# Research-Implementation/AudioVidSum-A-Multi-Modal-Approach-to-Video-Summarization

Hardware: AMD Instinct MI355X
Metric: frames/sec end-to-end (extract+fuse+score), 224x224 + 16kHz (higher is better)
Workload: dtype f16x2; 1 GPU; configs[1]: SumMe-shape batch, 25 videos x ~1800 frames (45143 frames/GPU), visual-only resnet50 extractor (batch-stat BN, the reference's 4-frame BatchNorm micro-batches inside each video) + AVBiLSTM attention scorer + mean-threshold selection; frames_per_gpu=45143, videos_per_gpu=25, extractor=resnet50, frames_per_group=4, chunk_frames=16384, parallelism=videos sharded x1, no data-path collective, selected_frames_rank0=22823

## Files before the change

audiovidsum-a-multi-modal-approach-to-video-summarization_amd/csrc/local224.hip:

```cpp
#include "avs_internal.h"
#include "igemm_params.h"
#include <type_traits>
#include <utility>

namespace {
constexpr int L_ROWS = 224;
constexpr int L_MT = L_ROWS / 32;
constexpr int L_BN = 128;
constexpr int L_CPRR = 4;
constexpr int L_STEP = 16;
constexpr int L_BUF = (L_ROWS + L_BN) * L_CPRR;
constexpr int L_P = 32 + 8;
constexpr unsigned L_OOB = 0x80000000u;

template <int OFF>
__device__ __forceinline__ uint4 lds_read_b128_at(unsigned byte_addr) {
  uint4 v;
  asm volatile("ds_read_b128 %0, %1 offset:%2" : "=v"(v) : "v"(byte_addr), "n"(OFF));
  return v;
}
template <int... I>
__device__ __forceinline__ void read_blocks(uint4 (&f)[L_MT], unsigned addr, std::integer_sequence<int, I...>) {
  ((f[I] = lds_read_b128_at<I * 32 * 64>(addr)), ...);
}
}

template <bool SPATIAL>
__global__ __launch_bounds__(256, 2) void igemm_h2_local224_kernel(IgemmParams p) {
  __shared__ uint4 lds[3 * L_BUF];

  const unsigned nwg = gridDim.x, orig = blockIdx.x;
  const unsigned q = nwg >> 3, rr = nwg & 7, xcd = orig & 7;
  const unsigned wg = (xcd < rr ? xcd * (q + 1) : rr * (q + 1) + (xcd - rr) * q) + (orig >> 3);
  int tn = wg % p.tiles_n;
  int tm = wg / p.tiles_n;
  if (p.packed) {
    const unsigned u_t = (unsigned)p.packed, tnn = (unsigned)p.tiles_n;
    const unsigned tiles_m = nwg / tnn;
    const unsigned full = (56u % u_t == 0u) ? (tiles_m / 56u) * 56u : 0u;
    if (orig < full * tnn) {
      const unsigned su = orig / (56u * tnn), l = orig - su * (56u * tnn);
      tn = (int)(l / 56u);
      tm = (int)(su * 56u + l % 56u);
    } else {
      const unsigned o2 = orig - full * tnn, unit = u_t * tnn;
      const unsigned u = o2 / unit, l = o2 - u * unit;
      const unsigned left = tiles_m - full - u * u_t, ul = left < u_t ? left : u_t;
      tn = (int)(l / ul);
      tm = (int)(full + u * u_t + l % ul);
    }
  } else if (p.cluster > 1) {
    const unsigned c = (unsigned)p.cluster, tnn = (unsigned)p.tiles_n;
    const unsigned tiles_m = nwg / tnn;
    const unsigned full = (8u % c == 0u) ? (tiles_m / 8u) * 8u : 0u;
    if (orig < full * tnn) {
      const unsigned su = orig / (8u * tnn), l = orig - su * (8u * tnn);
      tn = (int)(l >> 3);
      tm = (int)(su * 8u + (l & 7u));
    } else {
      const unsigned o2 = orig - full * tnn, unit = c * tnn;
      const unsigned u = o2 / unit, l = o2 - u * unit;
      tn = (int)(l / c);
      tm = (int)(full + u * c + l % c);
    }
  }
  const int m0 = tm * p.tile_rows;
  const int n0 = tn * L_BN;
  const int used = m0 + p.tile_rows <= p.M ? p.tile_rows : p.M - m0;

  const char* __restrict__ x = p.x;
  const char* __restrict__ w = p.w;
  char* __restrict__ y = p.y;

  const int t = threadIdx.x;
  const int wave = __builtin_amdgcn_readfirstlane(t >> 6), lane = t & 63;
  const bool extra = wave < 2;
  const int c = t & (L_CPRR - 1);
  const int rb = t >> 2;
  const int cq = c ^ ((rb >> 2) & (L_CPRR - 1));

  unsigned amask[4], aoff[4], boff[2];
  int f_tap = 0, f_ci0 = 0, f_kw = 0;
  int f_koff = 0;
  int f_kb = 0;
  __amdgpu_buffer_rsrc_t a_rsrc, b_rsrc;
  {
    const int taps = p.K / p.cin;
    long long a_origin;
    int n_first = 0;
    if (p.lin_stride >= 0) {
      a_origin = (long long)m0 * p.lin_stride;
    } else {
      n_first = m0 / p.HoWo;
      a_origin = (long long)n_first * p.x_img_stride - (long long)p.ph * p.x_row_stride - (long long)p.pw * p.x_px_stride;
    }
    a_rsrc = __builtin_amdgcn_make_buffer_rsrc(const_cast<char*>(x) + a_origin * 4, 0, (int)L_OOB, 0x00020000);
    b_rsrc = __builtin_amdgcn_make_buffer_rsrc(
        const_cast<char*>(w) + (p.w_kstep ? (long long)n0 * 64 : (long long)n0 * p.ldb * 4), 0, (int)L_OOB, 0x00020000);
#pragma unroll
    for (int i = 0; i < 4; ++i) {
      unsigned mk = 0, off = L_OOB;
      const int r = rb + 64 * i;
      if (r < used) {
        const int m = m0 + r;
        if (p.lin_stride >= 0) {
          mk = ~0u;
          off = (unsigned)((long long)r * p.lin_stride * 4) + cq * 16;
        } else {
          const int n = m / p.HoWo;
          const int rem = m - n * p.HoWo;
          const int ho = rem / p.Wo;
          const int wo = rem - ho * p.Wo;
          const int hi0 = ho * p.sh - p.ph, wi0 = wo * p.sw - p.pw;
          if constexpr (SPATIAL) {
            for (int tp = 0; tp < taps; ++tp) {
              const int th = tp / p.KW, tw = tp - th * p.KW;
              if ((unsigned)(hi0 + th) < (unsigned)p.H && (unsigned)(wi0 + tw) < (unsigned)p.W) mk |= 1u << tp;
            }
          } else {
            mk = ~0u;
          }
          off = (unsigned)(((long long)(n - n_first) * p.x_img_stride + (long long)(hi0 + p.ph) * p.x_row_stride +
                            (long long)(wi0 + p.pw) * p.x_px_stride) * 4) + cq * 16;
        }
      }
      amask[i] = mk;
      aoff[i] = off;
    }
#pragma unroll
    for (int i = 0; i < 2; ++i)
      boff[i] = p.w_kstep ? (unsigned)((rb + 64 * i) * 64) + (unsigned)(cq >> 2) * (unsigned)p.N * 64u + (cq & 3) * 16
                          : (unsigned)((long long)(rb + 64 * i) * p.ldb * 4) + cq * 16;
  }

  auto stage = [&](int buf) {
    uint4* abuf = lds + buf * L_BUF + wave * 64;
    uint4* bbuf = abuf + L_ROWS * L_CPRR;
#pragma unroll
    for (int i = 0; i < 3; ++i) {
      unsigned off = aoff[i];
      if constexpr (SPATIAL) off = ((amask[i] >> f_tap) & 1u) ? off : L_OOB;
      __builtin_amdgcn_raw_ptr_buffer_load_lds(a_rsrc, (__attribute__((address_space(3))) void*)(abuf + 256 * i), 16,
                                               (int)off, f_koff, 0, 0);
    }
    if (extra) {
      unsigned off = aoff[3];
      if constexpr (SPATIAL) off = ((amask[3] >> f_tap) & 1u) ? off : L_OOB;
      __builtin_amdgcn_raw_ptr_buffer_load_lds(a_rsrc, (__attribute__((address_space(3))) void*)(abuf + 256 * 3), 16,
                                               (int)off, f_koff, 0, 0);
    }
#pragma unroll
    for (int i = 0; i < 2; ++i)
      __builtin_amdgcn_raw_ptr_buffer_load_lds(b_rsrc, (__attribute__((address_space(3))) void*)(bbuf + 256 * i), 16,
                                               (int)boff[i], f_kb, 0, 0);
    f_kb += p.w_kstep ? p.N * 64 : L_STEP * 4;
    f_ci0 += L_STEP;
    f_koff += L_STEP * 4;
    if (f_ci0 == p.cin) {
      f_ci0 = 0;
      ++f_tap;
      f_koff += (int)((p.x_px_stride - p.cin) * 4);
      if (++f_kw == p.KW) {
        f_kw = 0;
        f_koff += (int)((p.x_row_stride - (long long)p.KW * p.x_px_stride) * 4);
      }
    }
  };

  const int lr = lane & 31, lh = lane >> 5;

  f32x16 acc[L_MT];
#pragma unroll
  for (int i = 0; i < L_MT; ++i)
#pragma unroll
    for (int e = 0; e < 16; ++e) acc[i][e] = 0.f;

  const unsigned lds_base = (unsigned)(unsigned long long)((__attribute__((address_space(3))) char*)lds);
  unsigned fa_off[2], fb_off[2];
#pragma unroll
  for (int hl = 0; hl < 2; ++hl) {
    const int chunk = 2 * lh + hl;
    fa_off[hl] = (unsigned)(lr * L_CPRR + (chunk ^ ((lr >> 2) & (L_CPRR - 1)))) * 16u;
    const int brow = wave * 32 + lr;
    fb_off[hl] = (unsigned)((L_ROWS + brow) * L_CPRR + (chunk ^ ((brow >> 2) & (L_CPRR - 1)))) * 16u;
  }

  const int col = n0 + wave * 32 + lr;
  const float inv_n = 1.f / (float)p.tile_rows;
  const int lim = used - 4 * lh;
  const int rl0 = lane >> 2, grp = lane & 3;
  const int col8 = n0 + wave * 32 + grp * 8;
  constexpr int DEPTH = 6;
  uint4 rhi[DEPTH][2], rlo[DEPTH][2];
  auto res_fetch = [&](auto blk) {
    constexpr int mt = decltype(blk)::value;
    const long long row0 = (long long)m0 + mt * 32 + rl0;
    const char* base = p.residual + (row0 * p.ldr + col8) * 4;
#pragma unroll
    for (int it = 0; it < 2; ++it) {
      const bool ok = mt * 32 + rl0 + 16 * it < used;
      const uint4* rp = reinterpret_cast<const uint4*>(ok ? base + (long long)it * 16 * p.ldr * 4 : p.residual);
      rhi[mt % DEPTH][it] = rp[0];
      rlo[mt % DEPTH][it] = rp[1];
    }
  };
  if (p.residual) {
    res_fetch(std::integral_constant<int, 0>{});
    res_fetch(std::integral_constant<int, 1>{});
    res_fetch(std::integral_constant<int, 2>{});
  }

  const int steps = p.K / L_STEP;
  stage(0);
  if (steps > 1) stage(1);
  int cur = 0;
  for (int s = 0; s < steps; ++s) {
    if (s + 1 < steps) {
      if (extra)
        asm volatile("s_waitcnt vmcnt(6)" ::: "memory");
      else
        asm volatile("s_waitcnt vmcnt(5)" ::: "memory");
    } else {
      asm volatile("s_waitcnt vmcnt(0)" ::: "memory");
    }
    __builtin_amdgcn_s_barrier();
    const unsigned bbase = lds_base + (unsigned)cur * (L_BUF * 16u);
    uint4 fah[L_MT], fal[L_MT], fbh, fbl;
    fbh = avs_lds_read_b128(bbase + fb_off[0]);
    read_blocks(fah, bbase + fa_off[0], std::make_integer_sequence<int, L_MT>{});
    fbl = avs_lds_read_b128(bbase + fb_off[1]);
    read_blocks(fal, bbase + fa_off[1], std::make_integer_sequence<int, L_MT>{});
    if (s + 2 < steps) stage(cur == 0 ? 2 : cur - 1);
    asm volatile("s_waitcnt lgkmcnt(%0)" ::"n"(1 + L_MT) : "memory");
    avs_pin(fbh);
#pragma unroll
    for (int mt = 0; mt < L_MT; ++mt) avs_pin(fah[mt]);
    __builtin_amdgcn_sched_barrier(0);
#pragma unroll
    for (int mt = 0; mt < L_MT; ++mt)
      acc[mt] = __builtin_amdgcn_mfma_f32_32x32x16_f16(__builtin_bit_cast(avs_f16x8, fah[mt]),
                                                       __builtin_bit_cast(avs_f16x8, fbh), acc[mt], 0, 0, 0);
    asm volatile("s_waitcnt lgkmcnt(0)" ::: "memory");
    avs_pin(fbl);
#pragma unroll
    for (int mt = 0; mt < L_MT; ++mt) avs_pin(fal[mt]);
    __builtin_amdgcn_sched_barrier(0);
#pragma unroll
    for (int mt = 0; mt < L_MT; ++mt) {
      acc[mt] = __builtin_amdgcn_mfma_f32_32x32x16_f16(__builtin_bit_cast(avs_f16x8, fal[mt]),
                                                       __builtin_bit_cast(avs_f16x8, fbh), acc[mt], 0, 0, 0);
      acc[mt] = __builtin_amdgcn_mfma_f32_32x32x16_f16(__builtin_bit_cast(avs_f16x8, fah[mt]),
                                                       __builtin_bit_cast(avs_f16x8, fbl), acc[mt], 0, 0, 0);
    }
    __builtin_amdgcn_sched_barrier(0);
    cur = cur == 2 ? 0 : cur + 1;
  }

  if (p.residual) {
    res_fetch(std::integral_constant<int, 3>{});
    res_fetch(std::integral_constant<int, 4>{});
    res_fetch(std::integral_constant<int, 5>{});
  }
  const int seg0 = p.packed ? (int)min((long long)used, (m0 / p.rows_per_group + 1ll) * p.rows_per_group - m0) : used;
  const bool shared = seg0 < used;
  float mean, mean_b, s2, s2b = 0.f;
  if (p.packed) {
    float s1 = 0.f, s1b = 0.f;
#pragma unroll
    for (int mt = 0; mt < L_MT; ++mt)
#pragma unroll
      for (int e = 0; e < 16; ++e) {
        if (mt < 3 || (mt == 3 && e < 8))
          s1 += acc[mt][e];
        else
          s1b += acc[mt][e];
      }
    s1 += __shfl_xor(s1, 32, 64);
    s1b += __shfl_xor(s1b, 32, 64);
    const float inv0 = 1.f / (float)seg0, inv1 = 1.f / (float)(shared ? used - seg0 : seg0);
    mean = (shared ? s1 : s1 + s1b) * inv0;
    mean_b = shared ? s1b * inv1 : mean;
    s2 = 0.f;
#pragma unroll
    for (int mt = 0; mt < L_MT; ++mt)
#pragma unroll
      for (int e = 0; e < 16; ++e) {
        const int roff = mt * 32 + (e & 3) + 8 * (e >> 2);
        if (mt < 3 || (mt == 3 && e < 8)) {
          const float d = acc[mt][e] - mean;
          s2 = roff < lim ? fmaf(d, d, s2) : s2;
        } else {
          const float d = acc[mt][e] - mean_b;
          s2b = roff < lim ? fmaf(d, d, s2b) : s2b;
        }
      }
    s2 += __shfl_xor(s2, 32, 64);
    s2b += __shfl_xor(s2b, 32, 64);
    if (!shared) s2 += s2b;
  } else {
    float s1 = 0.f;
#pragma unroll
    for (int mt = 0; mt < L_MT; ++mt)
#pragma unroll
      for (int e = 0; e < 16; ++e) s1 += acc[mt][e];
    s1 += __shfl_xor(s1, 32, 64);
    mean = mean_b = s1 * inv_n;
    s2 = 0.f;
#pragma unroll
    for (int mt = 0; mt < L_MT; ++mt)
#pragma unroll
      for (int e = 0; e < 16; ++e) {
        const int roff = mt * 32 + (e & 3) + 8 * (e >> 2);
        const float d = acc[mt][e] - mean;
        s2 = roff < lim ? fmaf(d, d, s2) : s2;
      }
    s2 += __shfl_xor(s2, 32, 64);
  }
  float g_mean = mean, g_var = s2 * inv_n;
  float g_mean_b = 0.f, g_var_b = 0.f;
  if (p.packed) {
    const long long gstride = (long long)p.tiles_n * 4 * 2 * 64;
    unsigned long long* const cbase = p.xchg + ((long long)tn * 4 + wave) * 2 * 64;
    unsigned long long* slot = cbase + tm * gstride + lane;
    __hip_atomic_store(slot, ((unsigned long long)p.epoch << 32) | (unsigned long long)__float_as_uint(lh ? s2 : mean),
                       __ATOMIC_RELAXED, __HIP_MEMORY_SCOPE_AGENT);
    if (shared)
      __hip_atomic_store(slot + 64, ((unsigned long long)p.epoch << 32) | (unsigned long long)__float_as_uint(lh ? s2b : mean_b),
                         __ATOMIC_RELAXED, __HIP_MEMORY_SCOPE_AGENT);
    const long long rpg = p.rows_per_group;
    const long long g0 = m0 / rpg;
#pragma unroll 1
    for (int sg = 0; sg <= (shared ? 1 : 0); ++sg) {
      const long long f0 = (g0 + sg) * rpg;
      const int tf = (int)(f0 / L_ROWS), tl = (int)((f0 + rpg - 1) / L_ROWS);
      float n = 0.f, mu = 0.f, m2 = 0.f;
      for (int j0 = tf; j0 <= tl; j0 += 4) {
        unsigned long long g[4];
        auto granule = [&](int j) { return cbase + (j * gstride + ((long long)j * L_ROWS < f0 ? 64 : 0)) + lane; };
#pragma unroll
        for (int u = 0; u < 4; ++u)
          g[u] = __hip_atomic_load(granule(j0 + u <= tl ? j0 + u : tm), __ATOMIC_RELAXED, __HIP_MEMORY_SCOPE_AGENT);
#pragma unroll
        for (int u = 0; u < 4; ++u) {
          const int j = j0 + u;
          if (j > tl) break;
          const long long lo = max(f0, (long long)j * L_ROWS), hi = min(f0 + rpg, (long long)(j + 1) * L_ROWS);
          const float nt = (float)(hi - lo);
          bool ok = (unsigned)(g[u] >> 32) == p.epoch;
#pragma unroll 1
          for (int spin = 0; spin < (1 << 20) && __builtin_amdgcn_read_exec() != __builtin_amdgcn_ballot_w64(ok); ++spin) {
            __builtin_amdgcn_s_sleep(8);
            g[u] = __hip_atomic_load(granule(j), __ATOMIC_RELAXED, __HIP_MEMORY_SCOPE_AGENT);
            ok = (unsigned)(g[u] >> 32) == p.epoch;
          }
          if (__builtin_amdgcn_read_exec() != __builtin_amdgcn_ballot_w64(ok) && lane == 0) atomicAdd(p.xerr, 1u);
          const float v = __uint_as_float((unsigned)g[u]);
          const float o = __shfl_xor(v, 32, 64);
          const float mj = lh ? o : v, qj = lh ? v : o;
          const float tot = n + nt, delta = mj - mu;
          mu += delta * (nt / tot);
          m2 += qj + delta * delta * (n * nt / tot);
          n = tot;
        }
      }
      const float gv = m2 / n;
      if (sg) {
        g_mean_b = mu;
        g_var_b = gv;
      } else {
        g_mean = mu;
        g_var = gv;
      }
    }
  } else if (p.cluster > 1) {
    const int cj = tm % p.cluster, t0 = tm - cj;
    unsigned long long* slot = p.xchg + (((long long)tm * p.tiles_n + tn) * 4 + wave) * 64 + lane;
    const float mine = lh ? s2 : mean;
    __hip_atomic_store(slot, ((unsigned long long)p.epoch << 32) | (unsigned long long)__float_as_uint(mine), __ATOMIC_RELAXED,
                       __HIP_MEMORY_SCOPE_AGENT);
    const float nt = (float)p.tile_rows;
    float n = 0.f, mu = 0.f, m2 = 0.f;
    const unsigned long long* const gbase = p.xchg + (((long long)t0 * p.tiles_n + tn) * 4 + wave) * 64 + lane;
    const long long gstride = (long long)p.tiles_n * 4 * 64;
    for (int j0 = 0; j0 < p.cluster; j0 += 4) {
      unsigned long long g[4];
#pragma unroll
      for (int u = 0; u < 4; ++u) {
        const int j = j0 + u < p.cluster ? j0 + u : cj;
        g[u] = __hip_atomic_load(gbase + j * gstride, __ATOMIC_RELAXED, __HIP_MEMORY_SCOPE_AGENT);
      }
#pragma unroll
      for (int u = 0; u < 4; ++u) {
        const int j = j0 + u;
        if (j >= p.cluster) break;
        float mj = mean, qj = s2;
        if (j != cj) {
          bool ok = (unsigned)(g[u] >> 32) == p.epoch;
          for (int spin = 0; spin < (1 << 20) && __builtin_amdgcn_read_exec() != __builtin_amdgcn_ballot_w64(ok); ++spin) {
            __builtin_amdgcn_s_sleep(8);
            g[u] = __hip_atomic_load(gbase + j * gstride, __ATOMIC_RELAXED, __HIP_MEMORY_SCOPE_AGENT);
            ok = (unsigned)(g[u] >> 32) == p.epoch;
          }
          if (__builtin_amdgcn_read_exec() != __builtin_amdgcn_ballot_w64(ok) && lane == 0) atomicAdd(p.xerr, 1u);
          const float v = __uint_as_float((unsigned)g[u]);
          const float o = __shfl_xor(v, 32, 64);
          mj = lh ? o : v;
          qj = lh ? v : o;
        }
        const float tot = n + nt, delta = mj - mu;
        mu += delta * (nt / tot);
        m2 += qj + delta * delta * (n * nt / tot);
        n = tot;
      }
    }
    g_mean = mu;
    g_var = m2 / n;
  }
  const float sc = p.gamma[col] / sqrtf(g_var + p.eps);
  const float sf = p.beta[col] - g_mean * sc;
  float sc_b = sc, sf_b = sf;
  if (shared) {
    sc_b = p.gamma[col] / sqrtf(g_var_b + p.eps);
    sf_b = p.beta[col] - g_mean_b * sc_b;
  }
#pragma unroll
  for (int mt = 0; mt < L_MT; ++mt)
#pragma unroll
    for (int e = 0; e < 16; ++e) {
      const bool first = mt < 3 || (mt == 3 && e < 8);
      acc[mt][e] = fmaf(acc[mt][e], first ? sc : sc_b, first ? sf : sf_b);
    }
  const bool relu = p.act == AVS_ACT_RELU;

  __syncthreads();
  float* const wreg = reinterpret_cast<float*>(lds) + wave * (32 * L_P);
  auto emit = [&](auto blk) {
    constexpr int mt = decltype(blk)::value;
#pragma unroll
    for (int e = 0; e < 16; ++e) wreg[((e & 3) + 8 * (e >> 2) + 4 * lh) * L_P + lr] = acc[mt][e];
    asm volatile("s_waitcnt lgkmcnt(0)" ::: "memory");
    __builtin_amdgcn_wave_barrier();
    const long long row0 = (long long)m0 + mt * 32 + rl0;
    char* const ybase = y + (row0 * p.ldc + col8) * 4;
#pragma unroll
    for (int it = 0; it < 2; ++it) {
      const float* src = wreg + (rl0 + 16 * it) * L_P + grp * 8;
      const float4 f0 = *reinterpret_cast<const float4*>(src);
      const float4 f1 = *reinterpret_cast<const float4*>(src + 4);
      if (!(mt * 32 + rl0 + 16 * it < used)) continue;
      float v[8] = {f0.x, f0.y, f0.z, f0.w, f1.x, f1.y, f1.z, f1.w};
      if (p.residual) {
        float rv[8];
        avs_pin(rhi[mt % DEPTH][it]);
        avs_pin(rlo[mt % DEPTH][it]);
        avs_f16x2_join8(rhi[mt % DEPTH][it], rlo[mt % DEPTH][it], rv);
#pragma unroll
        for (int j = 0; j < 8; ++j) v[j] += rv[j];
      }
      if (relu) {
#pragma unroll
        for (int j = 0; j < 8; ++j) v[j] = fmaxf(v[j], 0.f);
      }
      uint4 hi, lo;
      avs_f16x2_split8(v, hi, lo);
      uint4* dst = reinterpret_cast<uint4*>(ybase + (long long)it * 16 * p.ldc * 4);
      dst[0] = hi;
      dst[1] = lo;
    }
    asm volatile("s_waitcnt lgkmcnt(0)" ::: "memory");
    __builtin_amdgcn_wave_barrier();
    if constexpr (mt + DEPTH < L_MT) {
      if (p.residual) res_fetch(std::integral_constant<int, mt + DEPTH>{});
    }
  };
  emit(std::integral_constant<int, 0>{});
  emit(std::integral_constant<int, 1>{});
  emit(std::integral_constant<int, 2>{});
  emit(std::integral_constant<int, 3>{});
  emit(std::integral_constant<int, 4>{});
  emit(std::integral_constant<int, 5>{});
  emit(std::integral_constant<int, 6>{});
}

bool igemm_h2_local224_ok(const IgemmParams& p, int dtype, long long lin_stride) {
  const int tile_mode = p.variant & 3;
  if (dtype != AVS_F16X2 || !(tile_mode == AVS_TILE_AUTO || tile_mode == AVS_TILE_224)) return false;
  if (p.variant & AVS_STAGING_GENERIC) return false;
  const int cl = p.cluster > 1 ? p.cluster : 1;
  if (p.packed) {
    if (p.tile_rows != L_ROWS || p.cluster <= 1 || p.rows_per_group < L_ROWS || p.rows_per_group % (L_ROWS / 2) != 0) return false;
  } else if (p.tile_rows * cl != p.rows_per_group || p.tile_rows <= 192 || p.tile_rows > L_ROWS) {
    return false;
  }
  if (p.N % L_BN != 0 || p.M % p.rows_per_group != 0) return false;
  if (p.cin % L_STEP != 0 || p.K % L_STEP != 0 || p.K % p.cin != 0 || p.K / p.cin > 32) return false;
  return igemm_buffer_window_ok(p, lin_stride, 4, L_BN);
}

void igemm_h2_local224_launch(const IgemmParams& p, bool spatial, dim3 grid, hipStream_t stream) {
  if (spatial)
    hipLaunchKernelGGL(igemm_h2_local224_kernel<true>, grid, dim3(256), 0, stream, p);
  else
    hipLaunchKernelGGL(igemm_h2_local224_kernel<false>, grid, dim3(256), 0, stream, p);
}
```

Baseline: 27910 frames/s.

## Use 16x16x32 MFMA path with split-K LDS reads for pointwise local224 convs

Adds a SHAPE template parameter to the local224 implicit-GEMM kernel and a new 16x16x32 f16 MFMA main loop with re-swizzled LDS fragment offsets. The loop pairs even and odd K-steps and uses exec-masked half-wave LDS reads so fragments load in pieces between MFMA groups. The BN statistics, scale/shift and epilogue are adapted to the 16x16 accumulator layout. Pointwise (non-spatial) convolutions now use the 16 shape by default while spatial ones keep 32x32, aiming for better MFMA throughput and latency hiding at the cost of more complex scheduling and register pressure.

```diff
diff --git a/audiovidsum-a-multi-modal-approach-to-video-summarization_amd/csrc/local224.hip b/audiovidsum-a-multi-modal-approach-to-video-summarization_amd/csrc/local224.hip
--- a/audiovidsum-a-multi-modal-approach-to-video-summarization_amd/csrc/local224.hip
+++ b/audiovidsum-a-multi-modal-approach-to-video-summarization_amd/csrc/local224.hip
@@ -23,10 +23,67 @@
 __device__ __forceinline__ void read_blocks(uint4 (&f)[L_MT], unsigned addr, std::integer_sequence<int, I...>) {
   ((f[I] = lds_read_b128_at<I * 32 * 64>(addr)), ...);
 }
-}
-
-template <bool SPATIAL>
+
+typedef float f32x4 __attribute__((ext_vector_type(4)));
+constexpr int L_MT16 = L_ROWS / 16;
+template <int... I>
+__device__ __forceinline__ void read_blocks16(uint4 (&f)[L_MT16], unsigned addr, std::integer_sequence<int, I...>) {
+  ((f[I] = lds_read_b128_at<I * 16 * 64>(addr)), ...);
+}
+template <int B0, bool UPPER>
+__device__ __forceinline__ void read_half7(uint4 (&f)[L_MT16], unsigned addr) {
+  u32x4 r0 = __builtin_bit_cast(u32x4, f[B0 + 0]), r1 = __builtin_bit_cast(u32x4, f[B0 + 1]),
+        r2 = __builtin_bit_cast(u32x4, f[B0 + 2]), r3 = __builtin_bit_cast(u32x4, f[B0 + 3]),
+        r4 = __builtin_bit_cast(u32x4, f[B0 + 4]), r5 = __builtin_bit_cast(u32x4, f[B0 + 5]),
+        r6 = __builtin_bit_cast(u32x4, f[B0 + 6]);
+  if constexpr (UPPER)
+    asm volatile(
+        "s_mov_b32 exec_lo, 0\n\t"
+        "ds_read_b128 %0, %7 offset:%8\n\tds_read_b128 %1, %7 offset:%9\n\tds_read_b128 %2, %7 offset:%10\n\t"
+        "ds_read_b128 %3, %7 offset:%11\n\tds_read_b128 %4, %7 offset:%12\n\tds_read_b128 %5, %7 offset:%13\n\t"
+        "ds_read_b128 %6, %7 offset:%14\n\t"
+        "s_mov_b32 exec_lo, -1"
+        : "+v"(r0), "+v"(r1), "+v"(r2), "+v"(r3), "+v"(r4), "+v"(r5), "+v"(r6)
+        : "v"(addr), "n"((B0 + 0) * 1024), "n"((B0 + 1) * 1024), "n"((B0 + 2) * 1024), "n"((B0 + 3) * 1024),
+          "n"((B0 + 4) * 1024), "n"((B0 + 5) * 1024), "n"((B0 + 6) * 1024));
+  else
+    asm volatile(
+        "s_mov_b32 exec_hi, 0\n\t"
+        "ds_read_b128 %0, %7 offset:%8\n\tds_read_b128 %1, %7 offset:%9\n\tds_read_b128 %2, %7 offset:%10\n\t"
+        "ds_read_b128 %3, %7 offset:%11\n\tds_read_b128 %4, %7 offset:%12\n\tds_read_b128 %5, %7 offset:%13\n\t"
+        "ds_read_b128 %6, %7 offset:%14\n\t"
+        "s_mov_b32 exec_hi, -1"
+        : "+v"(r0), "+v"(r1), "+v"(r2), "+v"(r3), "+v"(r4), "+v"(r5), "+v"(r6)
+        : "v"(addr), "n"((B0 + 0) * 1024), "n"((B0 + 1) * 1024), "n"((B0 + 2) * 1024), "n"((B0 + 3) * 1024),
+          "n"((B0 + 4) * 1024), "n"((B0 + 5) * 1024), "n"((B0 + 6) * 1024));
+  f[B0 + 0] = __builtin_bit_cast(uint4, r0); f[B0 + 1] = __builtin_bit_cast(uint4, r1);
+  f[B0 + 2] = __builtin_bit_cast(uint4, r2); f[B0 + 3] = __builtin_bit_cast(uint4, r3);
+  f[B0 + 4] = __builtin_bit_cast(uint4, r4); f[B0 + 5] = __builtin_bit_cast(uint4, r5);
+  f[B0 + 6] = __builtin_bit_cast(uint4, r6);
+}
+__device__ __forceinline__ void read_upper2(uint4 (&f)[2], unsigned addr) {
+  u32x4 r0 = __builtin_bit_cast(u32x4, f[0]), r1 = __builtin_bit_cast(u32x4, f[1]);
+  asm volatile(
+      "s_mov_b32 exec_lo, 0\n\t"
+      "ds_read_b128 %0, %2\n\tds_read_b128 %1, %2 offset:1024\n\t"
+      "s_mov_b32 exec_lo, -1"
+      : "+v"(r0), "+v"(r1)
+      : "v"(addr));
+  f[0] = __builtin_bit_cast(uint4, r0);
+  f[1] = __builtin_bit_cast(uint4, r1);
+}
+__device__ __forceinline__ void zero_upper(uint4& f) {
+  asm volatile(
+      "s_mov_b32 exec_lo, 0\n\t"
+      "v_mov_b32 %0, 0\n\tv_mov_b32 %1, 0\n\tv_mov_b32 %2, 0\n\tv_mov_b32 %3, 0\n\t"
+      "s_mov_b32 exec_lo, -1"
+      : "+v"(f.x), "+v"(f.y), "+v"(f.z), "+v"(f.w));
+}
+}
+
+template <bool SPATIAL, int SHAPE>
 __global__ __launch_bounds__(256, 2) void igemm_h2_local224_kernel(IgemmParams p) {
+  static_assert(SHAPE == 32 || SHAPE == 16, "SHAPE: 32 (v_mfma_f32_32x32x16_f16) or 16 (v_mfma_f32_16x16x32_f16)");
   __shared__ uint4 lds[3 * L_BUF];
 
   const unsigned nwg = gridDim.x, orig = blockIdx.x;
@@ -170,10 +227,34 @@
   const int lr = lane & 31, lh = lane >> 5;
 
   f32x16 acc[L_MT];
-#pragma unroll
-  for (int i = 0; i < L_MT; ++i)
-#pragma unroll
-    for (int e = 0; e < 16; ++e) acc[i][e] = 0.f;
+  f32x4 acc16[L_MT16][2];
+  if constexpr (SHAPE == 32) {
+#pragma unroll
+    for (int i = 0; i < L_MT; ++i)
+#pragma unroll
+      for (int e = 0; e < 16; ++e) acc[i][e] = 0.f;
+  } else {
+#pragma unroll
+    for (int i = 0; i < L_MT16; ++i)
+#pragma unroll
+      for (int cb = 0; cb < 2; ++cb)
+#pragma unroll
+        for (int e = 0; e < 4; ++e) acc16[i][cb][e] = 0.f;
+  }
+  const int li = lane & 15, lg = lane >> 4;
+  const int rho = li ^ ((li >> 1) & 4);
+  const int rgp = lg ^ (lg >> 1);
+  unsigned fa16_even, fa16_odd, fb16_p, fb16_q;
+  {
+    const int hk = 2 * (lg & 1);
+    const int sw = (rho >> 2) & (L_CPRR - 1);
+    fa16_even = (unsigned)(rho * L_CPRR + ((hk + (lg >> 1)) ^ sw)) * 16u;
+    fa16_odd = (unsigned)(rho * L_CPRR + ((hk + 1 - (lg >> 1)) ^ sw)) * 16u;
+    const int brow = wave * 32 + li;
+    const int swb = (brow >> 2) & (L_CPRR - 1);
+    fb16_p = (unsigned)((L_ROWS + brow) * L_CPRR + (hk ^ swb)) * 16u;
+    fb16_q = (unsigned)((L_ROWS + brow) * L_CPRR + ((hk + 1) ^ swb)) * 16u;
+  }
 
   const unsigned lds_base = (unsigned)(unsigned long long)((__attribute__((address_space(3))) char*)lds);
   unsigned fa_off[2], fb_off[2];
@@ -207,56 +288,165 @@
   if (p.residual) {
     res_fetch(std::integral_constant<int, 0>{});
     res_fetch(std::integral_constant<int, 1>{});
-    res_fetch(std::integral_constant<int, 2>{});
+    if constexpr (SHAPE == 32) res_fetch(std::integral_constant<int, 2>{});
   }
 
   const int steps = p.K / L_STEP;
   stage(0);
   if (steps > 1) stage(1);
   int cur = 0;
-  for (int s = 0; s < steps; ++s) {
-    if (s + 1 < steps) {
-      if (extra)
-        asm volatile("s_waitcnt vmcnt(6)" ::: "memory");
-      else
-        asm volatile("s_waitcnt vmcnt(5)" ::: "memory");
-    } else {
-      asm volatile("s_waitcnt vmcnt(0)" ::: "memory");
-    }
-    __builtin_amdgcn_s_barrier();
-    const unsigned bbase = lds_base + (unsigned)cur * (L_BUF * 16u);
-    uint4 fah[L_MT], fal[L_MT], fbh, fbl;
-    fbh = avs_lds_read_b128(bbase + fb_off[0]);
-    read_blocks(fah, bbase + fa_off[0], std::make_integer_sequence<int, L_MT>{});
-    fbl = avs_lds_read_b128(bbase + fb_off[1]);
-    read_blocks(fal, bbase + fa_off[1], std::make_integer_sequence<int, L_MT>{});
-    if (s + 2 < steps) stage(cur == 0 ? 2 : cur - 1);
-    asm volatile("s_waitcnt lgkmcnt(%0)" ::"n"(1 + L_MT) : "memory");
-    avs_pin(fbh);
-#pragma unroll
-    for (int mt = 0; mt < L_MT; ++mt) avs_pin(fah[mt]);
-    __builtin_amdgcn_sched_barrier(0);
-#pragma unroll
-    for (int mt = 0; mt < L_MT; ++mt)
-      acc[mt] = __builtin_amdgcn_mfma_f32_32x32x16_f16(__builtin_bit_cast(avs_f16x8, fah[mt]),
-                                                       __builtin_bit_cast(avs_f16x8, fbh), acc[mt], 0, 0, 0);
-    asm volatile("s_waitcnt lgkmcnt(0)" ::: "memory");
-    avs_pin(fbl);
-#pragma unroll
-    for (int mt = 0; mt < L_MT; ++mt) avs_pin(fal[mt]);
-    __builtin_amdgcn_sched_barrier(0);
-#pragma unroll
-    for (int mt = 0; mt < L_MT; ++mt) {
-      acc[mt] = __builtin_amdgcn_mfma_f32_32x32x16_f16(__builtin_bit_cast(avs_f16x8, fal[mt]),
-                                                       __builtin_bit_cast(avs_f16x8, fbh), acc[mt], 0, 0, 0);
-      acc[mt] = __builtin_amdgcn_mfma_f32_32x32x16_f16(__builtin_bit_cast(avs_f16x8, fah[mt]),
-                                                       __builtin_bit_cast(avs_f16x8, fbl), acc[mt], 0, 0, 0);
-    }
-    __builtin_amdgcn_sched_barrier(0);
-    cur = cur == 2 ? 0 : cur + 1;
+  if constexpr (SHAPE == 32) {
+    for (int s = 0; s < steps; ++s) {
+      if (s + 1 < steps) {
+        if (extra)
+          asm volatile("s_waitcnt vmcnt(6)" ::: "memory");
+        else
+          asm volatile("s_waitcnt vmcnt(5)" ::: "memory");
+      } else {
+        asm volatile("s_waitcnt vmcnt(0)" ::: "memory");
+      }
+      __builtin_amdgcn_s_barrier();
+      const unsigned bbase = lds_base + (unsigned)cur * (L_BUF * 16u);
+      uint4 fah[L_MT], fal[L_MT], fbh, fbl;
+      fbh = avs_lds_read_b128(bbase + fb_off[0]);
+      read_blocks(fah, bbase + fa_off[0], std::make_integer_sequence<int, L_MT>{});
+      fbl = avs_lds_read_b128(bbase + fb_off[1]);
+      read_blocks(fal, bbase + fa_off[1], std::make_integer_sequence<int, L_MT>{});
+      if (s + 2 < steps) stage(cur == 0 ? 2 : cur - 1);
+      asm volatile("s_waitcnt lgkmcnt(%0)" ::"n"(1 + L_MT) : "memory");
+      avs_pin(fbh);
+  #pragma unroll
+      for (int mt = 0; mt < L_MT; ++mt) avs_pin(fah[mt]);
+      __builtin_amdgcn_sched_barrier(0);
+  #pragma unroll
+      for (int mt = 0; mt < L_MT; ++mt)
+        acc[mt] = __builtin_amdgcn_mfma_f32_32x32x16_f16(__builtin_bit_cast(avs_f16x8, fah[mt]),
+                                                         __builtin_bit_cast(avs_f16x8, fbh), acc[mt], 0, 0, 0);
+      asm volatile("s_waitcnt lgkmcnt(0)" ::: "memory");
+      avs_pin(fbl);
+  #pragma unroll
+      for (int mt = 0; mt < L_MT; ++mt) avs_pin(fal[mt]);
+      __builtin_amdgcn_sched_barrier(0);
+  #pragma unroll
+      for (int mt = 0; mt < L_MT; ++mt) {
+        acc[mt] = __builtin_amdgcn_mfma_f32_32x32x16_f16(__builtin_bit_cast(avs_f16x8, fal[mt]),
+                                                         __builtin_bit_cast(avs_f16x8, fbh), acc[mt], 0, 0, 0);
+        acc[mt] = __builtin_amdgcn_mfma_f32_32x32x16_f16(__builtin_bit_cast(avs_f16x8, fah[mt]),
+                                                         __builtin_bit_cast(avs_f16x8, fbl), acc[mt], 0, 0, 0);
+      }
+      __builtin_amdgcn_sched_barrier(0);
+      cur = cur == 2 ? 0 : cur + 1;
+    }
+  } else {
+    auto step_wait = [&](int s) {
+      if (s + 1 < steps) {
+        if (extra)
+          asm volatile("s_waitcnt vmcnt(6)" ::: "memory");
+        else
+          asm volatile("s_waitcnt vmcnt(5)" ::: "memory");
+      } else {
+        asm volatile("s_waitcnt vmcnt(0)" ::: "memory");
+      }
+      __builtin_amdgcn_s_barrier();
+    };
+    auto mfma_blocks = [&](auto first, const uint4 (&a)[L_MT16], const uint4 (&b)[2]) {
+      constexpr int b0 = decltype(first)::value;
+#pragma unroll
+      for (int mt = b0; mt < b0 + 7; ++mt)
+#pragma unroll
+        for (int cb = 0; cb < 2; ++cb)
+          acc16[mt][cb] = __builtin_amdgcn_mfma_f32_16x16x32_f16(__builtin_bit_cast(avs_f16x8, a[mt]),
+                                                                 __builtin_bit_cast(avs_f16x8, b[cb]), acc16[mt][cb], 0, 0, 0);
+    };
+    auto pin7 = [&](auto first, uint4 (&a)[L_MT16]) {
+      constexpr int b0 = decltype(first)::value;
+#pragma unroll
+      for (int mt = b0; mt < b0 + 7; ++mt) avs_pin(a[mt]);
+    };
+    constexpr std::integral_constant<int, 0> B0{};
+    constexpr std::integral_constant<int, 7> B7{};
+    uint4 fa[L_MT16], fbp[2], fbq[2];
+    auto even_step = [&](int s) {
+      step_wait(s);
+      const unsigned bbase = lds_base + (unsigned)cur * (L_BUF * 16u);
+      fbp[0] = lds_read_b128_at<0>(bbase + fb16_p);
+      fbp[1] = lds_read_b128_at<1024>(bbase + fb16_p);
+      read_blocks16(fa, bbase + fa16_even, std::make_integer_sequence<int, L_MT16>{});
+      if (s + 2 < steps) stage(cur == 0 ? 2 : cur - 1);
+      asm volatile("s_waitcnt lgkmcnt(7)" ::: "memory");
+      avs_pin(fbp[0]);
+      avs_pin(fbp[1]);
+      pin7(B0, fa);
+      __builtin_amdgcn_sched_barrier(0);
+      mfma_blocks(B0, fa, fbp);
+      __builtin_amdgcn_sched_barrier(0);
+      fbq[0] = lds_read_b128_at<0>(bbase + fb16_q);
+      fbq[1] = lds_read_b128_at<1024>(bbase + fb16_q);
+      asm volatile("s_waitcnt lgkmcnt(2)" ::: "memory");
+      pin7(B7, fa);
+      __builtin_amdgcn_sched_barrier(0);
+      mfma_blocks(B7, fa, fbp);
+      __builtin_amdgcn_sched_barrier(0);
+      cur = cur == 2 ? 0 : cur + 1;
+    };
+    auto odd_step = [&](int s) {
+      step_wait(s);
+      const unsigned bbase = lds_base + (unsigned)cur * (L_BUF * 16u);
+      read_upper2(fbq, bbase + fb16_q);
+      read_half7<0, true>(fa, bbase + fa16_odd);
+      read_half7<7, true>(fa, bbase + fa16_odd);
+      if (s + 2 < steps) stage(cur == 0 ? 2 : cur - 1);
+      asm volatile("s_waitcnt lgkmcnt(7)" ::: "memory");
+      avs_pin(fbq[0]);
+      avs_pin(fbq[1]);
+      pin7(B0, fa);
+      __builtin_amdgcn_sched_barrier(0);
+      mfma_blocks(B0, fa, fbq);
+      __builtin_amdgcn_sched_barrier(0);
+      read_half7<0, false>(fa, bbase + fa16_odd);
+      fbp[0] = lds_read_b128_at<0>(bbase + fb16_p);
+      fbp[1] = lds_read_b128_at<1024>(bbase + fb16_p);
+      asm volatile("s_waitcnt lgkmcnt(9)" ::: "memory");
+      pin7(B7, fa);
+      __builtin_amdgcn_sched_barrier(0);
+      mfma_blocks(B7, fa, fbq);
+      __builtin_amdgcn_sched_barrier(0);
+      read_half7<7, false>(fa, bbase + fa16_odd);
+      asm volatile("s_waitcnt lgkmcnt(7)" ::: "memory");
+      avs_pin(fbp[0]);
+      avs_pin(fbp[1]);
+      pin7(B0, fa);
+      __builtin_amdgcn_sched_barrier(0);
+      mfma_blocks(B0, fa, fbp);
+      __builtin_amdgcn_sched_barrier(0);
+      asm volatile("s_waitcnt lgkmcnt(0)" ::: "memory");
+      pin7(B7, fa);
+      __builtin_amdgcn_sched_barrier(0);
+      mfma_blocks(B7, fa, fbp);
+      __builtin_amdgcn_sched_barrier(0);
+      cur = cur == 2 ? 0 : cur + 1;
+    };
+    int s = 0;
+    for (; s + 1 < steps; s += 2) {
+      even_step(s);
+      odd_step(s + 1);
+    }
+    if (s < steps) {
+      even_step(s);
+      asm volatile("s_waitcnt lgkmcnt(0)" ::: "memory");
+      zero_upper(fbq[0]);
+      zero_upper(fbq[1]);
+#pragma unroll
+      for (int mt = 0; mt < L_MT16; ++mt) zero_upper(fa[mt]);
+      __builtin_amdgcn_sched_barrier(0);
+      mfma_blocks(B0, fa, fbq);
+      mfma_blocks(B7, fa, fbq);
+      __builtin_amdgcn_sched_barrier(0);
+    }
   }
 
   if (p.residual) {
+    if constexpr (SHAPE == 16) res_fetch(std::integral_constant<int, 2>{});
     res_fetch(std::integral_constant<int, 3>{});
     res_fetch(std::integral_constant<int, 4>{});
     res_fetch(std::integral_constant<int, 5>{});
@@ -264,7 +454,55 @@
   const int seg0 = p.packed ? (int)min((long long)used, (m0 / p.rows_per_group + 1ll) * p.rows_per_group - m0) : used;
   const bool shared = seg0 < used;
   float mean, mean_b, s2, s2b = 0.f;
-  if (p.packed) {
+  if constexpr (SHAPE == 16) {
+    const int lim16 = used - 4 * rgp;
+    const float inv0 = p.packed ? 1.f / (float)seg0 : inv_n, inv1 = 1.f / (float)(shared ? used - seg0 : seg0);
+    float mc[2], mbc[2], qc[2], qbc[2];
+#pragma unroll
+    for (int cb = 0; cb < 2; ++cb) {
+      float s1 = 0.f, s1b = 0.f;
+#pragma unroll
+      for (int mt = 0; mt < L_MT16; ++mt)
+#pragma unroll
+        for (int e = 0; e < 4; ++e) {
+          if (mt < L_MT16 / 2)
+            s1 += acc16[mt][cb][e];
+          else
+            s1b += acc16[mt][cb][e];
+        }
+      s1 += __shfl_xor(s1, 16, 64);
+      s1b += __shfl_xor(s1b, 16, 64);
+      s1 += __shfl_xor(s1, 32, 64);
+      s1b += __shfl_xor(s1b, 32, 64);
+      mc[cb] = (shared ? s1 : s1 + s1b) * inv0;
+      mbc[cb] = shared ? s1b * inv1 : mc[cb];
+      float q = 0.f, qb = 0.f;
+#pragma unroll
+      for (int mt = 0; mt < L_MT16; ++mt)
+#pragma unroll
+        for (int e = 0; e < 4; ++e) {
+          const int roff = mt * 16 + e;
+          if (mt < L_MT16 / 2) {
+            const float d = acc16[mt][cb][e] - mc[cb];
+            q = roff < lim16 ? fmaf(d, d, q) : q;
+          } else {
+            const float d = acc16[mt][cb][e] - mbc[cb];
+            qb = roff < lim16 ? fmaf(d, d, qb) : qb;
+          }
+        }
+      q += __shfl_xor(q, 16, 64);
+      qb += __shfl_xor(qb, 16, 64);
+      q += __shfl_xor(q, 32, 64);
+      qb += __shfl_xor(qb, 32, 64);
+      qc[cb] = shared ? q : q + qb;
+      qbc[cb] = qb;
+    }
+    const bool c1 = (lg & 1) != 0;
+    mean = c1 ? mc[1] : mc[0];
+    mean_b = c1 ? mbc[1] : mbc[0];
+    s2 = c1 ? qc[1] : qc[0];
+    s2b = c1 ? qbc[1] : qbc[0];
+  } else if (p.packed) {
     float s1 = 0.f, s1b = 0.f;
 #pragma unroll
     for (int mt = 0; mt < L_MT; ++mt)
@@ -423,21 +661,47 @@
     sc_b = p.gamma[col] / sqrtf(g_var_b + p.eps);
     sf_b = p.beta[col] - g_mean_b * sc_b;
   }
-#pragma unroll
-  for (int mt = 0; mt < L_MT; ++mt)
-#pragma unroll
-    for (int e = 0; e < 16; ++e) {
-      const bool first = mt < 3 || (mt == 3 && e < 8);
-      acc[mt][e] = fmaf(acc[mt][e], first ? sc : sc_b, first ? sf : sf_b);
-    }
+  if constexpr (SHAPE == 32) {
+#pragma unroll
+    for (int mt = 0; mt < L_MT; ++mt)
+#pragma unroll
+      for (int e = 0; e < 16; ++e) {
+        const bool first = mt < 3 || (mt == 3 && e < 8);
+        acc[mt][e] = fmaf(acc[mt][e], first ? sc : sc_b, first ? sf : sf_b);
+      }
+  } else {
+    const bool c1 = (lg & 1) != 0;
+    const float sc_o = __shfl_xor(sc, 16, 64), sf_o = __shfl_xor(sf, 16, 64);
+    const float scb_o = __shfl_xor(sc_b, 16, 64), sfb_o = __shfl_xor(sf_b, 16, 64);
+    const float sc2[2] = {c1 ? sc_o : sc, c1 ? sc : sc_o}, sf2[2] = {c1 ? sf_o : sf, c1 ? sf : sf_o};
+    const float scb2[2] = {c1 ? scb_o : sc_b, c1 ? sc_b : scb_o}, sfb2[2] = {c1 ? sfb_o : sf_b, c1 ? sf_b : sfb_o};
+#pragma unroll
+    for (int mt = 0; mt < L_MT16; ++mt)
+#pragma unroll
+      for (int cb = 0; cb < 2; ++cb)
+#pragma unroll
+        for (int e = 0; e < 4; ++e) {
+          const bool first = mt < L_MT16 / 2;
+          acc16[mt][cb][e] = fmaf(acc16[mt][cb][e], first ? sc2[cb] : scb2[cb], first ? sf2[cb] : sfb2[cb]);
+        }
+  }
   const bool relu = p.act == AVS_ACT_RELU;
 
   __syncthreads();
   float* const wreg = reinterpret_cast<float*>(lds) + wave * (32 * L_P);
   auto emit = [&](auto blk) {
     constexpr int mt = decltype(blk)::value;
-#pragma unroll
-    for (int e = 0; e < 16; ++e) wreg[((e & 3) + 8 * (e >> 2) + 4 * lh) * L_P + lr] = acc[mt][e];
+    if constexpr (SHAPE == 32) {
+#pragma unroll
+      for (int e = 0; e < 16; ++e) wreg[((e & 3) + 8 * (e >> 2) + 4 * lh) * L_P + lr] = acc[mt][e];
+    } else {
+#pragma unroll
+      for (int h = 0; h < 2; ++h)
+#pragma unroll
+        for (int cb = 0; cb < 2; ++cb)
+#pragma unroll
+          for (int e = 0; e < 4; ++e) wreg[(h * 16 + 4 * rgp + e) * L_P + cb * 16 + li] = acc16[2 * mt + h][cb][e];
+    }
     asm volatile("s_waitcnt lgkmcnt(0)" ::: "memory");
     __builtin_amdgcn_wave_barrier();
     const long long row0 = (long long)m0 + mt * 32 + rl0;
@@ -497,9 +761,26 @@
   return igemm_buffer_window_ok(p, lin_stride, 4, L_BN);
 }
 
+constexpr int L_SHAPE_SPATIAL = 32;
+constexpr int L_SHAPE_POINT = 16;
+
 void igemm_h2_local224_launch(const IgemmParams& p, bool spatial, dim3 grid, hipStream_t stream) {
+#ifdef AVS_STUDY
+  const int forced = getenv("AVS_LOCAL224_MFMA") ? atoi(getenv("AVS_LOCAL224_MFMA")) : 0;
+  if (forced == 16 || forced == 32) {
+    if (spatial && forced == 16)
+      hipLaunchKernelGGL((igemm_h2_local224_kernel<true, 16>), grid, dim3(256), 0, stream, p);
+    else if (spatial)
+      hipLaunchKernelGGL((igemm_h2_local224_kernel<true, 32>), grid, dim3(256), 0, stream, p);
+    else if (forced == 16)
+      hipLaunchKernelGGL((igemm_h2_local224_kernel<false, 16>), grid, dim3(256), 0, stream, p);
+    else
+      hipLaunchKernelGGL((igemm_h2_local224_kernel<false, 32>), grid, dim3(256), 0, stream, p);
+    return;
+  }
+#endif
   if (spatial)
-    hipLaunchKernelGGL(igemm_h2_local224_kernel<true>, grid, dim3(256), 0, stream, p);
+    hipLaunchKernelGGL((igemm_h2_local224_kernel<true, L_SHAPE_SPATIAL>), grid, dim3(256), 0, stream, p);
   else
-    hipLaunchKernelGGL(igemm_h2_local224_kernel<false>, grid, dim3(256), 0, stream, p);
-}
+    hipLaunchKernelGGL((igemm_h2_local224_kernel<false, L_SHAPE_POINT>), grid, dim3(256), 0, stream, p);
+}
```

After: 28190 frames/s, median of 6. +1.0%, better.
